# LambdaLabsML/distributed-training-guide

Measured on AMD Instinct MI355X. Metric: tokens/sec/GPU for Llama-style causal LM at 1/2/4/8 MI355X; peak HBM per GPU, higher is better.
Workload: dtype bf16; 1 GPU; model=llama-3-8b, global_batch=24, seq_len=1024, parallelism=single

## Files before the change

### distributed_training_guide_amd/_hip/attention_bwd.hip

```cpp
#include "attention_common.h"
#include "launchers.h"

template <int D>
__global__ void __launch_bounds__(256) attn_delta_kernel(
    const short* __restrict__ dout, const short* __restrict__ o,
    float* __restrict__ delta, int B, int S, int Hq) {
  const int grp = threadIdx.x >> 4;
  const int gl = threadIdx.x & 15;
  int64_t nrows = (int64_t)B * S * Hq;
  for (int64_t row = (int64_t)blockIdx.x * 16 + grp; row < nrows;
       row += (int64_t)gridDim.x * 16) {
    const short* dp = dout + row * D;
    const short* op = o + row * D;
    float s = 0.f;
#pragma unroll
    for (int i = gl * 8; i < D; i += 16 * 8) {
      bf16x8 dv = *reinterpret_cast<const bf16x8*>(dp + i);
      bf16x8 ov = *reinterpret_cast<const bf16x8*>(op + i);
#pragma unroll
      for (int j = 0; j < 8; ++j) s += bf2f(dv[j]) * bf2f(ov[j]);
    }
#pragma unroll
    for (int off = 1; off < 16; off <<= 1) s += __shfl_xor(s, off, WAVE);
    if (gl == 0) {
      int h = (int)(row % Hq);
      int64_t bs = row / Hq;
      int sp = (int)(bs % S);
      int b = (int)(bs / S);
      delta[((int64_t)b * Hq + h) * S + sp] = s;
    }
  }
}

template <int D, bool DOC>
__global__ void __launch_bounds__(256, 2) attn_dkdv_kernel(
    const short* __restrict__ dout, const short* __restrict__ q,
    const short* __restrict__ k, const short* __restrict__ v,
    const float* __restrict__ lse, const float* __restrict__ delta,
    short* __restrict__ dk, short* __restrict__ dv, int B, int S, int Hq,
    int Hkv, float scale, const int* __restrict__ doc_end) {
  static_assert(D == 64 || D == 128, "head dim must be 64 or 128");
  __shared__ short q_lds[2][64 * D];
  __shared__ short do_lds[2][64 * D];
  __shared__ __attribute__((aligned(16))) float lse_lds[2][64];
  __shared__ __attribute__((aligned(16))) float del_lds[2][64];

  const int nkt = (S + 63) / 64;
  const int group = Hq / Hkv;

  const GroupBlock gb = xcd_remap(blockIdx.x, B * Hkv, nkt);
  const int b = gb.gid / Hkv;
  const int hkv = gb.gid % Hkv;
  const int kt = gb.within;

  const int tid = threadIdx.x;
  const int wid = tid >> 6;
  const int lane = tid & (WAVE - 1);
  const int l15 = lane & 15;
  const int lg = lane >> 4;

  const int kv0 = kt * 64 + wid * 16;
  constexpr int nd16 = D >> 4, nkc = D >> 5;
  const float c2 = scale * LOG2E;
  const int64_t strideS_q = (int64_t)Hq * D;
  const int64_t strideS_kv = (int64_t)Hkv * D;
// ... 130 lines not shown
    for (int dt = 0; dt < nd16; ++dt) {
#pragma unroll
      for (int kc = 0; kc < 2; ++kc) {
        bf16x8 dofr = tr16_frag_st(dol, kc * 32 + lg * 8, dt * 16, l15);
        bf16x8 qfr = tr16_frag_st(ql, kc * 32 + lg * 8, dt * 16, l15);
        dvacc[dt] = mfma16(__builtin_bit_cast(bf16x8, pk_p[kc]), dofr,
                           dvacc[dt]);
        dkacc[dt] = mfma16(__builtin_bit_cast(bf16x8, pk_ds[kc]), qfr,
                           dkacc[dt]);
      }
    }
    __builtin_amdgcn_s_setprio(0);
    __syncthreads();
  }

#pragma unroll
  for (int r = 0; r < 4; ++r) {
    int keyw = kv0 + lg * 4 + r;
    if (keyw >= S) continue;
    short* dkp = dk + ((int64_t)b * S * Hkv + (int64_t)keyw * Hkv + hkv) * D;
    short* dvp = dv + ((int64_t)b * S * Hkv + (int64_t)keyw * Hkv + hkv) * D;
#pragma unroll
    for (int dt = 0; dt < nd16; ++dt) {
      dkp[dt * 16 + l15] = f2bf(dkacc[dt][r]);
      dvp[dt * 16 + l15] = f2bf(dvacc[dt][r]);
    }
  }
}

template <int D, bool DOC>
__global__ void __launch_bounds__(256, 2) attn_dq_kernel(
    const short* __restrict__ dout, const short* __restrict__ q,
    const short* __restrict__ k, const short* __restrict__ v,
    const float* __restrict__ lse, const float* __restrict__ delta,
    short* __restrict__ dq, int B, int S, int Hq, int Hkv, float scale,
    const int* __restrict__ doc_start) {
  static_assert(D == 64 || D == 128, "head dim must be 64 or 128");
  __shared__ short k_lds[2][KVBLK * D];
  __shared__ short v_lds[2][KVBLK * D];

  const int ntq = (S + QBLK - 1) / QBLK;
  const int gqa = Hq / Hkv;
  const int bpg = gqa * ntq;

  const GroupBlock gb = xcd_remap(blockIdx.x, B * Hkv, bpg);
  const int b = gb.gid / Hkv;
  const int hkv = gb.gid % Hkv;
  const int h = hkv * gqa + gb.within / ntq;
  const int qtile = gb.within % ntq;

  const int tid = threadIdx.x;
  const int wid = tid >> 6;
  const int lane = tid & (WAVE - 1);
  const int l15 = lane & 15;
  const int lg = lane >> 4;

  const int q0 = qtile * QBLK;
  const int rowb[2] = {qgroup_row(q0, wid, 0), qgroup_row(q0, wid, 1)};
  constexpr int nd16 = D >> 4, nkc = D >> 5;
  const float c2 = scale * LOG2E;
  const int64_t strideS_q = (int64_t)Hq * D;
  const int64_t strideS_kv = (int64_t)Hkv * D;
  const short* qb = q + ((int64_t)b * S * Hq + h) * D;
  const short* dob = dout + ((int64_t)b * S * Hq + h) * D;
  const short* kb = k + ((int64_t)b * S * Hkv + hkv) * D;
  const short* vb = v + ((int64_t)b * S * Hkv + hkv) * D;
  const float* lseb = lse + ((int64_t)b * Hq + h) * S;
  const float* delb = delta + ((int64_t)b * Hq + h) * S;

  bf16x8 qf[2][nkc], dof[2][nkc];
  float lse_r[2], del_r[2];
#pragma unroll
  for (int nq = 0; nq < 2; ++nq) {
    int qrow = rowb[nq] + l15;
    int qrc = qrow < S ? qrow : S - 1;
    const short* qp = qb + (int64_t)qrc * strideS_q + lg * 8;
    const short* dop = dob + (int64_t)qrc * strideS_q + lg * 8;
#pragma unroll
    for (int c = 0; c < nkc; ++c) {
      qf[nq][c] = *reinterpret_cast<const bf16x8*>(qp + c * 32);
      dof[nq][c] = *reinterpret_cast<const bf16x8*>(dop + c * 32);
    }
    lse_r[nq] = lseb[qrc] * LOG2E;
    del_r[nq] = delb[qrc] * scale;
  }

  f32x4 dqacc[nd16][2];
#pragma unroll
  for (int dt = 0; dt < nd16; ++dt)
#pragma unroll
    for (int nq = 0; nq < 2; ++nq) dqacc[dt][nq] = {0.f, 0.f, 0.f, 0.f};

  const int kv_end = min(S, q0 + QBLK);
  const int ntiles = (kv_end + KVBLK - 1) / KVBLK;
  int dstart[2], dsmax[2];
  const int t0 =
      doc_window<DOC>(doc_start, b, S, q0, wid, l15, dstart, dsmax);

  auto stage_kv = [&](int t, int buf) {
    stage_tile_pair<D>(kb, vb, strideS_kv, t * KVBLK, S, k_lds[buf],
                       v_lds[buf], wid, lane);
  };
  stage_kv(t0, 0);
  __syncthreads();

  for (int t = t0; t < ntiles; ++t) {
    const int kv0 = t * KVBLK;
    const int buf = tile_buf(t, t0);
    if (t + 1 < ntiles) stage_kv(t + 1, buf ^ 1);

    {
      const bool smask = (kv_end < kv0 + KVBLK);
      u32x4 pk_ds[2][2];
      const short* kl = k_lds[buf];
      const short* vl = v_lds[buf];
      __builtin_amdgcn_s_setprio(1);
#pragma unroll
// ... 31 lines not shown
              const int keyr = kv0 + koff + r;
              if (keyr > qrow || keyr >= S || qrow >= S ||
                  (DOC && keyr < dstart[nq]))
                e[r] = -INFINITY;
            }
          }
#pragma unroll
          for (int r = 0; r < 4; ++r)
            ds[r] = __builtin_amdgcn_exp2f(e[r]) *
                    __builtin_fmaf(dv[r], scale, -del_r[nq]);
          pk_ds[nq][kc][rp + 0] = cvt_pk_bf16(ds[0], ds[1]);
          pk_ds[nq][kc][rp + 1] = cvt_pk_bf16(ds[2], ds[3]);
        }
      }

#pragma unroll
      for (int dt = 0; dt < nd16; ++dt) {
#pragma unroll
        for (int kc = 0; kc < 2; ++kc) {
          bf16x8 kfr = tr16_frag_st(kl, kc * 32 + lg * 8, dt * 16, l15);
          dqacc[dt][0] = mfma16(__builtin_bit_cast(bf16x8, pk_ds[0][kc]),
                                kfr, dqacc[dt][0]);
          dqacc[dt][1] = mfma16(__builtin_bit_cast(bf16x8, pk_ds[1][kc]),
                                kfr, dqacc[dt][1]);
        }
      }
      __builtin_amdgcn_s_setprio(0);
    }
    __syncthreads();
  }

#pragma unroll
  for (int nq = 0; nq < 2; ++nq) {
#pragma unroll
    for (int r = 0; r < 4; ++r) {
      int qrow = rowb[nq] + lg * 4 + r;
      if (qrow >= S) continue;
      short* dqp = dq + ((int64_t)b * S * Hq + (int64_t)qrow * Hq + h) * D;
#pragma unroll
      for (int dt = 0; dt < nd16; ++dt) {
        dqp[dt * 16 + l15] = f2bf(dqacc[dt][nq][r]);
      }
    }
  }
}

namespace {
template <int D, bool DOC>
void bwd_launch(const short* dout, const short* q, const short* k,
                const short* v, const short* o, const float* lse,
                float* delta, short* dq, short* dk, short* dv,
                const int* doc_start, const int* doc_end, int B, int S,
                int Hq, int Hkv, float scale, hipStream_t stream) {
  int64_t nrows = (int64_t)B * S * Hq;
  int64_t dwant = (nrows + 15) / 16;
  int dgrid = (int)(dwant < 2048 ? (dwant < 1 ? 1 : dwant) : 2048);
  hipLaunchKernelGGL(attn_delta_kernel<D>, dim3(dgrid), dim3(256), 0, stream,
                     dout, o, delta, B, S, Hq);
  int nkt = (S + 63) / 64;
  hipLaunchKernelGGL((attn_dkdv_kernel<D, DOC>),
                     dim3((uint32_t)((int64_t)B * Hkv * nkt)), dim3(256), 0,
                     stream, dout, q, k, v, lse, delta, dk, dv, B, S, Hq, Hkv,
                     scale, doc_end);
  int ntq = (S + QBLK - 1) / QBLK;
  hipLaunchKernelGGL((attn_dq_kernel<D, DOC>),
                     dim3((uint32_t)((int64_t)B * Hq * ntq)), dim3(256), 0,
                     stream, dout, q, k, v, lse, delta, dq, B, S, Hq, Hkv,
                     scale, doc_start);
}
}

extern "C" void attn_bwd_launch(const void* dout, const void* q, const void* k,
                                const void* v, const void* o, const float* lse,
                                float* delta, void* dq, void* dk, void* dv,
                                const int* doc_start, const int* doc_end,
                                int B, int S, int Hq, int Hkv, int D,
                                float scale, hipStream_t stream) {
  const bool doc = doc_start != nullptr;
  auto fn = doc ? (D == 64 ? bwd_launch<64, true> : bwd_launch<128, true>)
                : (D == 64 ? bwd_launch<64, false> : bwd_launch<128, false>);
  fn((const short*)dout, (const short*)q, (const short*)k, (const short*)v,
     (const short*)o, lse, delta, (short*)dq, (short*)dk, (short*)dv,
     doc_start, doc_end, B, S, Hq, Hkv, scale, stream);
}
```

### distributed_training_guide_amd/_hip/bindings.cpp

```cpp
#include <torch/extension.h>
#include <c10/hip/HIPStream.h>
#include <hip/hip_runtime.h>

#include "launchers.h"

namespace {

inline hipStream_t cur_stream() {
  return c10::hip::getCurrentHIPStream().stream();
}

#define CHECK_BF16_CONTIG(t)                                          \
  TORCH_CHECK((t).is_cuda(), #t " must be on the GPU");               \
  TORCH_CHECK((t).dtype() == torch::kBFloat16, #t " must be bf16");   \
  TORCH_CHECK((t).is_contiguous(), #t " must be contiguous")

#define CHECK_ROPE_TABLES(cos, sin, x, D)                                  \
  TORCH_CHECK((D) % 2 == 0, "rope head dim must be even");                 \
  TORCH_CHECK((cos).is_cuda() && (cos).device() == (x).device() &&         \
                  (sin).is_cuda() && (sin).device() == (x).device(),       \
              "rope tables must be on " #x "'s device");                   \
  TORCH_CHECK((cos).dtype() == torch::kFloat &&                            \
                  (sin).dtype() == torch::kFloat,                          \
              "rope tables must be f32");                                  \
// ... 197 lines not shown
  TORCH_CHECK(dy.sizes() == c10::IntArrayRef(sizes),
              "dy must have gu's shape with the last dim halved");
  TORCH_CHECK(dy.device() == gu.device(), "dy must be on gu's device");
  auto dgu = torch::empty_like(gu);
  silu_mul_bwd_launch(dy.data_ptr(), gu.data_ptr(), dgu.data_ptr(),
                      gu.numel() / I2, I, cur_stream());
  return dgu;
}

torch::Tensor embedding_fwd(torch::Tensor table, torch::Tensor ids) {
  CHECK_BF16_CONTIG(table);
  TORCH_CHECK(table.dim() == 2, "table must be [V,H]");
  TORCH_CHECK(ids.is_cuda() && ids.device() == table.device(),
              "ids must be on the table's device");
  TORCH_CHECK(ids.dtype() == torch::kLong && ids.is_contiguous());
  const int64_t V = table.size(0);
  const int H = (int)table.size(1);
  auto sizes = ids.sizes().vec();
  sizes.push_back(H);
  auto out = torch::empty(sizes, table.options());
  embed_fwd_launch(table.data_ptr(), ids.data_ptr<int64_t>(),
                   out.data_ptr(), ids.numel(), H, V, cur_stream());
  return out;
}

torch::Tensor embedding_bwd(torch::Tensor dy, torch::Tensor ids, int64_t V) {
  CHECK_BF16_CONTIG(dy);
  TORCH_CHECK(ids.is_cuda() && ids.device() == dy.device(),
              "ids must be on dy's device");
  TORCH_CHECK(ids.dtype() == torch::kLong && ids.is_contiguous());
  TORCH_CHECK(dy.dim() >= 1 && V > 0, "dy must be [..., H] and V positive");
  const int H = (int)dy.size(-1);
  TORCH_CHECK(dy.numel() == ids.numel() * H, "dy/ids shape mismatch");
  auto acc = torch::empty({V, (int64_t)H},
                          dy.options().dtype(torch::kFloat));
  auto dtable = torch::empty({V, (int64_t)H}, dy.options());
  embed_bwd_launch(dy.data_ptr(), ids.data_ptr<int64_t>(),
                   acc.data_ptr<float>(), dtable.data_ptr(), ids.numel(), H,
                   V, cur_stream());
  return dtable;
}

std::vector<torch::Tensor> layernorm_fwd(torch::Tensor x, torch::Tensor w,
                                         torch::Tensor b, double eps) {
  CHECK_BF16_CONTIG(x);
  CHECK_BF16_CONTIG(w);
  CHECK_BF16_CONTIG(b);
  const int H = (int)x.size(-1);
  const int64_t nrows = x.numel() / H;
  auto y = torch::empty_like(x);
  auto opts = x.options().dtype(torch::kFloat);
  auto mu = torch::empty({nrows}, opts);
  auto rstd = torch::empty({nrows}, opts);
  ln_fwd_launch(x.data_ptr(), w.data_ptr(), b.data_ptr(), y.data_ptr(),
                mu.data_ptr<float>(), rstd.data_ptr<float>(), nrows, H,
                (float)eps, cur_stream());
  return {y, mu, rstd};
}

std::vector<torch::Tensor> layernorm_bwd(torch::Tensor dy, torch::Tensor x,
                                         torch::Tensor w, torch::Tensor mu,
                                         torch::Tensor rstd) {
  CHECK_BF16_CONTIG(dy);
  CHECK_BF16_CONTIG(x);
  const int H = (int)x.size(-1);
  const int64_t nrows = x.numel() / H;
  const int nblocks = (int)std::min<int64_t>(nrows, 2048);
  auto dx = torch::empty_like(x);
  auto dw = torch::empty_like(w);
  auto db = torch::empty_like(w);
  auto dw_partial = alloc_partials(nblocks, H, x);
  auto db_partial = alloc_partials(nblocks, H, x);
// ... 31 lines not shown
  const int B = (int)logits.size(0), S = (int)logits.size(1),
            V = (int)logits.size(2);
  const int64_t nrows = (int64_t)B * S_out;
  auto loss = torch::empty({nrows}, logits.options().dtype(torch::kFloat));
  auto lse = torch::empty({nrows}, logits.options().dtype(torch::kFloat));
  ce_fwd_launch(logits.data_ptr(), labels.data_ptr<int64_t>(),
                loss.data_ptr<float>(), lse.data_ptr<float>(), nrows, S,
                (int)S_out, V, ignore_index, cur_stream());
  return {loss, lse};
}

std::vector<torch::Tensor> ce_fwd_sharded(torch::Tensor logits,
                                          torch::Tensor labels, int64_t S_out,
                                          int64_t vocab_start,
                                          int64_t ignore_index) {
  CHECK_CE_INPUTS(logits, labels, S_out);
  const int B = (int)logits.size(0), S = (int)logits.size(1),
            V = (int)logits.size(2);
  const int64_t nrows = (int64_t)B * S_out;
  auto opts = logits.options().dtype(torch::kFloat);
  auto maxout = torch::empty({nrows}, opts);
  auto sumout = torch::empty({nrows}, opts);
  auto gathered = torch::empty({nrows}, opts);
  ce_fwd_sharded_launch(logits.data_ptr(), labels.data_ptr<int64_t>(),
                        maxout.data_ptr<float>(), sumout.data_ptr<float>(),
                        gathered.data_ptr<float>(), nrows, S, (int)S_out, V,
                        vocab_start, ignore_index, cur_stream());
  return {maxout, sumout, gathered};
}

torch::Tensor ce_bwd(torch::Tensor logits, torch::Tensor labels,
                     torch::Tensor lse, double scale, int64_t S_out,
                     int64_t vocab_start, int64_t ignore_index, bool sharded,
                     c10::optional<torch::Tensor> scale_t = c10::nullopt) {
  CHECK_CE_INPUTS(logits, labels, S_out);
  const int B = (int)logits.size(0), S = (int)logits.size(1),
            V = (int)logits.size(2);
  const int64_t nrows = (int64_t)B * S_out;
  TORCH_CHECK(lse.is_cuda() && lse.device() == logits.device() &&
                  lse.dtype() == torch::kFloat && lse.is_contiguous() &&
                  lse.numel() == nrows,
              "lse must be a contiguous f32 [B*S_out] on the logits' device");
  const float* sp = nullptr;
  if (scale_t.has_value()) {
    TORCH_CHECK(scale_t->dtype() == torch::kFloat && scale_t->is_cuda() &&
                scale_t->numel() == 1, "scale_t must be a cuda f32 scalar");
    sp = scale_t->data_ptr<float>();
  }
  auto dlogits = (S_out == S) ? torch::empty_like(logits)
                              : torch::zeros_like(logits);
  ce_bwd_launch(logits.data_ptr(), labels.data_ptr<int64_t>(),
                lse.data_ptr<float>(), dlogits.data_ptr(), (float)scale, sp,
                nrows, S, (int)S_out, V, vocab_start, ignore_index,
                sharded ? 1 : 0, cur_stream());
  return dlogits;
}

void adamw_step(torch::Tensor descs, int64_t nchunks, double lr, double beta1,
                double beta2, double eps, double wd, int64_t step) {
  TORCH_CHECK(descs.is_cuda() && descs.dtype() == torch::kLong &&
              descs.is_contiguous());
  const float bc1 = 1.0f - std::pow((float)beta1, (float)step);
  const float bc2 = 1.0f - std::pow((float)beta2, (float)step);
  adamw_launch(descs.data_ptr(), (int)nchunks, (float)lr, (float)beta1,
               (float)beta2, (float)eps, (float)wd, 1.0f / bc1, 1.0f / bc2,
               cur_stream());
}

#define CHECK_DESCS(descs, nchunks)                                        \
  TORCH_CHECK((descs).is_cuda() && (descs).dtype() == torch::kLong &&      \
              (descs).is_contiguous());                                    \
  TORCH_CHECK((nchunks) >= 0 && (descs).numel() >= 7 * (nchunks),          \
              "descriptor table shorter than nchunks")

#define CHECK_SQ_TOTAL(t, descs)                                           \
  TORCH_CHECK((t).is_cuda() && (t).dtype() == torch::kFloat &&             \
              (t).numel() == 1 && (t).device() == (descs).device(),        \
              #t " must be a cuda f32 scalar on the descriptors' device")

void adamw_step_clipped(torch::Tensor descs, int64_t nchunks, double lr,
                        double beta1, double beta2, double eps, double wd,
                        int64_t step, torch::Tensor sq_total,
                        double max_norm) {
// ... 138 lines not shown
                       scale);
}
std::vector<torch::Tensor> attn_bwd_doc(torch::Tensor dout, torch::Tensor q,
                                        torch::Tensor k, torch::Tensor v,
                                        torch::Tensor o, torch::Tensor lse,
                                        torch::Tensor doc_start,
                                        torch::Tensor doc_end, double scale) {
  return attn_bwd_impl(dout, q, k, v, o, lse, doc_start, doc_end, scale);
}

}

PYBIND11_MODULE(TORCH_EXTENSION_NAME, m) {
  m.def("rmsnorm_fwd", &rmsnorm_fwd);
  m.def("rmsnorm_bwd", &rmsnorm_bwd);
  m.def("rope", &rope);
  m.def("add_rmsnorm_fwd", &add_rmsnorm_fwd);
  m.def("add_rmsnorm_bwd", &add_rmsnorm_bwd);
  m.def("qkv_rope_fwd", &qkv_rope_fwd);
  m.def("qkv_rope_bwd", &qkv_rope_bwd);
  m.def("silu_mul_fwd", &silu_mul_fwd);
  m.def("silu_mul_bwd", &silu_mul_bwd);
  m.def("embedding_fwd", &embedding_fwd);
  m.def("embedding_bwd", &embedding_bwd);
  m.def("layernorm_fwd", &layernorm_fwd);
  m.def("layernorm_bwd", &layernorm_bwd);
  m.def("gelu_fwd", &gelu_fwd);
  m.def("gelu_bwd", &gelu_bwd);
  m.def("ce_fwd", &ce_fwd);
  m.def("ce_fwd_sharded", &ce_fwd_sharded);
  m.def("ce_bwd", &ce_bwd, py::arg("logits"), py::arg("labels"),
        py::arg("lse"), py::arg("scale"), py::arg("S_out"),
        py::arg("vocab_start"), py::arg("ignore_index"),
        py::arg("sharded"), py::arg("scale_t") = c10::nullopt);
  m.def("adamw_step", &adamw_step);
  m.def("adamw_step_clipped", &adamw_step_clipped);
  m.def("grad_sqsum", &grad_sqsum);
  m.def("grad_scale_", &grad_scale_);
  m.def("attn_fwd", &attn_fwd);
  m.def("attn_bwd", &attn_bwd);
  m.def("attn_fwd_doc", &attn_fwd_doc);
  m.def("attn_bwd_doc", &attn_bwd_doc);
}
```

### distributed_training_guide_amd/_hip/cross_entropy.hip

```cpp
#include "common.h"
#include "launchers.h"

template <bool SHARDED>
__global__ void __launch_bounds__(256) ce_fwd_kernel(
    const short* __restrict__ logits, const int64_t* __restrict__ labels,
    float* __restrict__ loss, float* __restrict__ lse,
    float* __restrict__ maxout,
    float* __restrict__ sumout,
    float* __restrict__ gathered,
    int64_t nrows, int S_logits, int S_out, int V,
    int64_t vocab_start, int64_t ignore_index) {
  __shared__ float scratch[8];
  for (int64_t r = blockIdx.x; r < nrows; r += gridDim.x) {
    int64_t b = r / S_out;
    int64_t s = r % S_out;
    const short* xr = logits + (b * S_logits + s) * V;
    int64_t label = labels[b * S_logits + s + (S_logits - S_out)];
    float m = -INFINITY, sum = 0.0f;
    for (int i = threadIdx.x * 8; i < V; i += blockDim.x * 8) {
      s16x8 v;
      if (i + 8 <= V) v = *reinterpret_cast<const s16x8*>(xr + i);
      else { for (int j = 0; j < 8; ++j) v[j] = (i + j < V) ? xr[i + j] : (short)0xff80;  }
#pragma unroll
      for (int j = 0; j < 8; ++j) {
// ... 3 lines not shown
        sum += __expf(f - m);
      }
    }
    float gm = block_reduce_max(m, scratch);
    sum = (m == -INFINITY) ? 0.0f : sum * __expf(m - gm);
    sum = block_reduce_sum(sum, scratch);
    if (threadIdx.x == 0) {
      if (SHARDED) {
        float g = -INFINITY;
        int64_t local = label - vocab_start;
        if (label != ignore_index && local >= 0 && local < V)
          g = bf2f(xr[local]);
        maxout[r] = gm;
        sumout[r] = sum;
        gathered[r] = g;
      } else {
        if (label == ignore_index) {
          loss[r] = 0.0f;
          lse[r] = -INFINITY;
        } else {
          DTGA_KERNEL_ASSERT(label >= 0 && label < V);
          float l = gm + __logf(sum);
          lse[r] = l;
          loss[r] = l - bf2f(xr[label]);
        }
      }
    }
    __syncthreads();
  }
}

template <bool SHARDED>
__global__ void __launch_bounds__(256) ce_bwd_kernel(
    const short* __restrict__ logits, const int64_t* __restrict__ labels,
    const float* __restrict__ lse, short* __restrict__ dlogits, float scale,
    const float* __restrict__ scale_ptr,
    int64_t nrows, int S_logits, int S_out, int V,
    int64_t vocab_start, int64_t ignore_index) {
  if (scale_ptr != nullptr) scale = scale_ptr[0];
  for (int64_t r = blockIdx.x; r < nrows; r += gridDim.x) {
    int64_t b = r / S_out;
    int64_t s = r % S_out;
    const short* xr = logits + (b * S_logits + s) * V;
    short* dxr = dlogits + (b * S_logits + s) * V;
    int64_t label = labels[b * S_logits + s + (S_logits - S_out)];
    float l = lse[r];
    bool ignored = (label == ignore_index) || (l == -INFINITY);
    if (!SHARDED) DTGA_KERNEL_ASSERT(ignored || (label >= 0 && label < V));
    int64_t local = label - vocab_start;
    for (int i = threadIdx.x * 8; i < V; i += blockDim.x * 8) {
      if (i + 8 <= V) {
        s16x8 v = *reinterpret_cast<const s16x8*>(xr + i);
        s16x8 o;
#pragma unroll
        for (int j = 0; j < 8; ++j) {
          float p = ignored ? 0.0f : __expf(bf2f(v[j]) - l);
          if (!ignored && (int64_t)(i + j) == local) p -= 1.0f;
          o[j] = f2bf(scale * p);
        }
        *reinterpret_cast<s16x8*>(dxr + i) = o;
      } else {
        for (int j = 0; i + j < V; ++j) {
          float p = ignored ? 0.0f : __expf(bf2f(xr[i + j]) - l);
          if (!ignored && (int64_t)(i + j) == local) p -= 1.0f;
          dxr[i + j] = f2bf(scale * p);
        }
      }
    }
// ... 42 lines not shown
```

### distributed_training_guide_amd/_hip/embedding.hip

```cpp
#include "common.h"
#include "launchers.h"

__global__ void __launch_bounds__(256) embed_fwd_kernel(
    const short* __restrict__ table, const int64_t* __restrict__ ids,
    short* __restrict__ out, int64_t nrows, int H, int64_t V) {
  const int wave = threadIdx.x / WAVE;
  const int lane = threadIdx.x % WAVE;
  const int waves = blockDim.x / WAVE;
  for (int64_t r = (int64_t)blockIdx.x * waves + wave; r < nrows;
       r += (int64_t)gridDim.x * waves) {
    int64_t id = ids[r];
    DTGA_KERNEL_ASSERT(id >= 0 && id < V);
    const short* src = table + id * H;
    short* dst = out + r * H;
    if ((H & 7) == 0) {
      for (int i = lane * 8; i < H; i += WAVE * 8)
        *reinterpret_cast<s16x8*>(dst + i) =
            *reinterpret_cast<const s16x8*>(src + i);
    } else {
      for (int i = lane; i < H; i += WAVE) dst[i] = src[i];
    }
  }
}

__global__ void __launch_bounds__(256) embed_bwd_scatter_kernel(
    const short* __restrict__ dy, const int64_t* __restrict__ ids,
    float* __restrict__ acc, int64_t nrows, int H, int64_t V) {
  const int wave = threadIdx.x / WAVE;
  const int lane = threadIdx.x % WAVE;
  const int waves = blockDim.x / WAVE;
  for (int64_t r = (int64_t)blockIdx.x * waves + wave; r < nrows;
       r += (int64_t)gridDim.x * waves) {
    int64_t id = ids[r];
    DTGA_KERNEL_ASSERT(id >= 0 && id < V);
    const short* src = dy + r * H;
    float* dst = acc + id * H;
    if ((H & 3) == 0) {
      for (int i = lane * 4; i < H; i += WAVE * 4) {
        s16x4 v = *reinterpret_cast<const s16x4*>(src + i);
#pragma unroll
        for (int j = 0; j < 4; ++j) atomicAdd(dst + i + j, bf2f(v[j]));
      }
    } else {
      for (int i = lane; i < H; i += WAVE) atomicAdd(dst + i, bf2f(src[i]));
    }
  }
}

__global__ void __launch_bounds__(256) f32_to_bf16_kernel(
    const float* __restrict__ src, short* __restrict__ dst, int64_t n) {
  for (int64_t i = ((int64_t)blockIdx.x * blockDim.x + threadIdx.x) * 4;
       i < n; i += (int64_t)gridDim.x * blockDim.x * 4) {
    if (i + 4 <= n) {
      f32x4 v = *reinterpret_cast<const f32x4*>(src + i);
      s16x4 o;
#pragma unroll
      for (int j = 0; j < 4; ++j) o[j] = f2bf(v[j]);
      *reinterpret_cast<s16x4*>(dst + i) = o;
    } else {
      for (int64_t j = i; j < n; ++j) dst[j] = f2bf(src[j]);
    }
  }
}

extern "C" {
void embed_fwd_launch(const void* table, const int64_t* ids, void* out,
                      int64_t nrows, int H, int64_t V, hipStream_t s) {
  int waves = 4;
  int64_t blocks = (nrows + waves - 1) / waves;
  int grid = (int)(blocks < 8192 ? (blocks < 1 ? 1 : blocks) : 8192);
  hipLaunchKernelGGL(embed_fwd_kernel, dim3(grid), dim3(256), 0, s,
                     (const short*)table, ids, (short*)out, nrows, H, V);
}
void embed_bwd_launch(const void* dy, const int64_t* ids, float* acc,
                      void* dtable, int64_t nrows, int H, int64_t V,
                      hipStream_t s) {
  hipMemsetAsync(acc, 0, (size_t)V * H * sizeof(float), s);
  int waves = 4;
  int64_t blocks = (nrows + waves - 1) / waves;
  int grid = (int)(blocks < 8192 ? (blocks < 1 ? 1 : blocks) : 8192);
  hipLaunchKernelGGL(embed_bwd_scatter_kernel, dim3(grid), dim3(256), 0, s,
                     (const short*)dy, ids, acc, nrows, H, V);
  int64_t n = V * (int64_t)H;
  int64_t cblocks = (n / 4 + 255) / 256;
  int cgrid = (int)(cblocks < 1 ? 1 : cblocks < 8192 ? cblocks : 8192);
  hipLaunchKernelGGL(f32_to_bf16_kernel, dim3(cgrid), dim3(256), 0, s,
                     acc, (short*)dtable, n);
}
}
```

### distributed_training_guide_amd/_hip/launchers.h

```cpp
#pragma once
#include <hip/hip_runtime.h>
#include <stdint.h>

#define COLSUM_RY 16

extern "C" {
void colsum_launch(float* partial, void* out, int nblocks, int H,
                   hipStream_t s);

void rmsnorm_fwd_launch(const void* x, const void* w, void* y, void* rstd,
                        int64_t nrows, int H, float eps, hipStream_t s);
void rmsnorm_bwd_launch(const void* dy, const void* x, const void* w,
                        const void* rstd, void* dx, float* dw_partial,
                        void* dw, int nblocks, int64_t nrows, int H,
                        hipStream_t s);
void add_rmsnorm_fwd_launch(const void* res, const void* delta, const void* w,
                            void* res_out, void* y, void* rstd, int64_t nrows,
                            int H, float eps, hipStream_t s);
void add_rmsnorm_bwd_launch(const void* dy, const void* dres_out,
                            const void* x, const void* w, const void* rstd,
                            void* dx, float* dw_partial, void* dw,
                            int nblocks, int64_t nrows, int H,
                            hipStream_t s);

void ln_fwd_launch(const void* x, const void* w, const void* b, void* y,
                   float* mu, float* rstd, int64_t nrows, int H, float eps,
                   hipStream_t s);
void ln_bwd_launch(const void* dy, const void* x, const void* w,
                   const float* mu, const float* rstd, void* dx,
                   float* dw_partial, float* db_partial, void* dw, void* db,
                   int nblocks, int64_t nrows, int H, hipStream_t s);
void gelu_fwd_launch(const void* x, void* y, int64_t n, hipStream_t s);
void gelu_bwd_launch(const void* dy, const void* x, void* dx, int64_t n,
                     hipStream_t s);

void rope_launch(const void* x, void* y, const float* cs, const float* sn,
                 const int* positions, int64_t total_rows, int S, int H, int D,
                 int backward, hipStream_t stream);
void qkv_rope_fwd_launch(const void* qkv, void* q, void* k, void* v,
                         const float* cs, const float* sn,
                         const int* positions, int64_t BS, int S, int Hq,
                         int Hkv, int D, hipStream_t stream);
void qkv_rope_bwd_launch(const void* dq, const void* dk, const void* dv,
                         void* dqkv, const float* cs, const float* sn,
                         const int* positions, int64_t BS, int S, int Hq,
                         int Hkv, int D, hipStream_t stream);

void silu_mul_fwd_launch(const void* gu, void* y, int64_t nrows, int I,
                         hipStream_t s);
void silu_mul_bwd_launch(const void* dy, const void* gu, void* dgu,
                         int64_t nrows, int I, hipStream_t s);

void embed_fwd_launch(const void* table, const int64_t* ids, void* out,
                      int64_t nrows, int H, int64_t V, hipStream_t s);
void embed_bwd_launch(const void* dy, const int64_t* ids, float* acc,
                      void* dtable, int64_t nrows, int H, int64_t V,
                      hipStream_t s);

void ce_fwd_launch(const void* logits, const int64_t* labels, float* loss,
                   float* lse, int64_t nrows, int S_logits, int S_out, int V,
                   int64_t ignore_index, hipStream_t st);
void ce_fwd_sharded_launch(const void* logits, const int64_t* labels,
                           float* maxout, float* sumout, float* gathered,
                           int64_t nrows, int S_logits, int S_out, int V,
                           int64_t vocab_start, int64_t ignore_index,
                           hipStream_t st);
void ce_bwd_launch(const void* logits, const int64_t* labels, const float* lse,
                   void* dlogits, float scale, const float* scale_ptr,
                   int64_t nrows, int S_logits, int S_out, int V,
                   int64_t vocab_start, int64_t ignore_index, int sharded,
                   hipStream_t st);

void adamw_launch(const void* descs, int nchunks, float lr, float beta1,
                  float beta2, float eps, float wd, float inv_bc1,
                  float inv_bc2, hipStream_t s);
void adamw_launch_clipped(const void* descs, int nchunks, float lr,
                          float beta1, float beta2, float eps, float wd,
                          float inv_bc1, float inv_bc2, const float* sq_total,
                          float max_norm, hipStream_t s);
void grad_sqsum_launch(const void* descs, int nchunks, float* partials,
                       float* out, int slot, hipStream_t s);
void grad_scale_launch(const void* descs, int nchunks, const float* sq_total,
                       float max_norm, hipStream_t s);

void attn_fwd_launch(const void* q, const void* k, const void* v, void* o,
                     float* lse, const int* doc_start, int B, int S, int Hq,
                     int Hkv, int D, float scale, hipStream_t stream);
void attn_bwd_launch(const void* dout, const void* q, const void* k,
                     const void* v, const void* o, const float* lse,
                     float* delta, void* dq, void* dk, void* dv,
// ... 4 lines not shown
```

### distributed_training_guide_amd/_hip/silu_mul.hip

```cpp
#include "common.h"
#include "launchers.h"

__global__ void __launch_bounds__(256) silu_mul_fwd_kernel(
    const short* __restrict__ gu, short* __restrict__ y, int64_t nrows,
    int I) {
  const int gwave = (blockIdx.x * blockDim.x + threadIdx.x) / WAVE;
  const int nwaves = gridDim.x * blockDim.x / WAVE;
  const int lane = threadIdx.x & (WAVE - 1);
  for (int64_t row = gwave; row < nrows; row += nwaves) {
    const short* g = gu + row * (2 * (int64_t)I);
    const short* u = g + I;
    short* yr = y + row * (int64_t)I;
    for (int i = lane * 8; i < I; i += WAVE * 8) {
      s16x8 gv = *reinterpret_cast<const s16x8*>(g + i);
      s16x8 uv = *reinterpret_cast<const s16x8*>(u + i);
      s16x8 o;
#pragma unroll
      for (int j = 0; j < 8; ++j) {
        float x = bf2f(gv[j]);
        float sig = 1.0f / (1.0f + __expf(-x));
        o[j] = f2bf(x * sig * bf2f(uv[j]));
      }
      *reinterpret_cast<s16x8*>(yr + i) = o;
    }
  }
}

__global__ void __launch_bounds__(256) silu_mul_bwd_kernel(
    const short* __restrict__ dy, const short* __restrict__ gu,
    short* __restrict__ dgu, int64_t nrows, int I) {
  const int gwave = (blockIdx.x * blockDim.x + threadIdx.x) / WAVE;
  const int nwaves = gridDim.x * blockDim.x / WAVE;
  const int lane = threadIdx.x & (WAVE - 1);
  for (int64_t row = gwave; row < nrows; row += nwaves) {
    const short* dyr = dy + row * (int64_t)I;
    const short* g = gu + row * (2 * (int64_t)I);
    const short* u = g + I;
    short* dg = dgu + row * (2 * (int64_t)I);
    short* du = dg + I;
    for (int i = lane * 8; i < I; i += WAVE * 8) {
      s16x8 dv = *reinterpret_cast<const s16x8*>(dyr + i);
      s16x8 gv = *reinterpret_cast<const s16x8*>(g + i);
      s16x8 uv = *reinterpret_cast<const s16x8*>(u + i);
      s16x8 og, ou;
#pragma unroll
      for (int j = 0; j < 8; ++j) {
        float x = bf2f(gv[j]);
        float sig = 1.0f / (1.0f + __expf(-x));
        float sx = x * sig;
        float d = bf2f(dv[j]);
        ou[j] = f2bf(d * sx);
        og[j] = f2bf(d * bf2f(uv[j]) * sig * (1.0f + x * (1.0f - sig)));
      }
      *reinterpret_cast<s16x8*>(dg + i) = og;
      *reinterpret_cast<s16x8*>(du + i) = ou;
    }
// ... 21 lines not shown
```

### distributed_training_guide_amd/ops/embedding.py

```python
import torch
import torch.nn as nn
import torch.nn.functional as F

from .._ext import ext, use_hip


class _EmbeddingFn(torch.autograd.Function):
    @staticmethod
    def forward(ctx, ids, weight):
        ctx.save_for_backward(ids)
        ctx.V = weight.shape[0]
        return ext().embedding_fwd(weight, ids)

    @staticmethod
    def backward(ctx, dy):
        (ids,) = ctx.saved_tensors
        dtable = ext().embedding_bwd(dy.contiguous(), ids, ctx.V)
        return None, dtable


class Embedding(nn.Module):

    def __init__(self, num_embeddings: int, embedding_dim: int, device=None,
                 dtype=None):
        super().__init__()
        self.num_embeddings = num_embeddings
        self.embedding_dim = embedding_dim
        self.weight = nn.Parameter(torch.empty(
            num_embeddings, embedding_dim, device=device, dtype=dtype))

    def reset_parameters(self):
        with torch.no_grad():
            if not self.weight.is_meta:
                self.weight.normal_()

    def forward(self, ids):
        import os

        if (use_hip(self.weight)
                and not os.environ.get("DTGA_TORCH_EMBED")
                and not torch.are_deterministic_algorithms_enabled()):
            return _EmbeddingFn.apply(ids.contiguous(), self.weight)
        return F.embedding(ids, self.weight)

    def extra_repr(self):
        return f"{self.num_embeddings}, {self.embedding_dim}"
```

### distributed_training_guide_amd/ops/fused_linear_ce.py

```python
import os

import torch

from .._ext import ext
from .cross_entropy import IGNORE_INDEX
from .reference import cross_entropy_ref


def _shifted_flat_labels(labels: torch.Tensor) -> torch.Tensor:
    B, S = labels.shape
    flat = labels.reshape(-1)
    out = torch.empty_like(flat)
    out[: B * S - 1] = flat[1:]
    out[B * S - 1:].fill_(IGNORE_INDEX)
    out.view(B, S)[:, S - 1].fill_(IGNORE_INDEX)
    return out.contiguous()


class _FusedLinearCEFn(torch.autograd.Function):
    @staticmethod
    def forward(ctx, x, weight, labels, chunk_rows, keep_logits):
        B, S, H = x.shape
        x2 = x.reshape(B * S, H)
        N = B * S
        shifted = _shifted_flat_labels(labels)
        n_valid = (shifted != IGNORE_INDEX).sum().clamp_min(1)
        logits = None
        if keep_logits:
            logits = torch.matmul(x2, weight.t())
            loss_rows, lse = ext().ce_fwd(logits.unsqueeze(0),
                                          shifted.unsqueeze(0), N,
                                          IGNORE_INDEX)
            loss_sum = loss_rows.sum()
        else:
            lse = torch.empty(N, dtype=torch.float32, device=x.device)
            loss_sum = torch.zeros((), dtype=torch.float32, device=x.device)
            wt = weight.t()
            for r0 in range(0, N, chunk_rows):
                r1 = min(r0 + chunk_rows, N)
                logits_c = torch.matmul(x2[r0:r1], wt)
                lc, lse_c = ext().ce_fwd(logits_c.unsqueeze(0),
                                         shifted[r0:r1].unsqueeze(0), r1 - r0,
                                         IGNORE_INDEX)
                loss_sum += lc.sum()
                lse[r0:r1] = lse_c
        if keep_logits:
            ctx.save_for_backward(x2, weight, shifted, lse, n_valid, logits)
        else:
            ctx.save_for_backward(x2, weight, shifted, lse, n_valid)
        ctx.chunk_rows = chunk_rows
        ctx.in_shape = (B, S, H)
        ctx.keep_logits = keep_logits
        return loss_sum / n_valid

    @staticmethod
    def backward(ctx, dloss):
        if ctx.keep_logits:
            x2, weight, shifted, lse, n_valid, logits = ctx.saved_tensors
        else:
            x2, weight, shifted, lse, n_valid = ctx.saved_tensors
            logits = None
        B, S, H = ctx.in_shape
        V = weight.shape[0]
        N = B * S
        scale_t = (dloss.detach() / n_valid).to(torch.float32) \
            .reshape(1).contiguous()
        dx2 = torch.empty_like(x2)
        one_chunk = ctx.chunk_rows >= N
        dw32 = None if one_chunk else torch.zeros(
            V, H, dtype=torch.float32, device=x2.device)
        dw = None
        wt = weight.t()
        for r0 in range(0, N, ctx.chunk_rows):
            r1 = min(r0 + ctx.chunk_rows, N)
            L = r1 - r0
            logits_c = (logits[r0:r1] if logits is not None
                        else torch.matmul(x2[r0:r1], wt))
            dlogits_c = ext().ce_bwd(logits_c.unsqueeze(0),
                                     shifted[r0:r1].unsqueeze(0),
                                     lse[r0:r1], 0.0, L, 0, IGNORE_INDEX,
                                     False, scale_t).squeeze(0)
            del logits_c
            torch.matmul(dlogits_c, weight, out=dx2[r0:r1])
            if one_chunk:
                dw = torch.matmul(dlogits_c.t(), x2[r0:r1])
            else:
                dw32.add_(torch.matmul(dlogits_c.t(), x2[r0:r1]))
        if dw is None:
            dw = dw32.to(weight.dtype)
        return (dx2.view(B, S, H), dw, None, None, None)


def fused_causal_lm_loss(x: torch.Tensor, weight: torch.Tensor,
                         labels: torch.Tensor,
                         chunk_rows: int | None = None) -> torch.Tensor:
    if not x.is_cuda:
        logits = torch.matmul(x, weight.t())
        return cross_entropy_ref(logits, labels, IGNORE_INDEX)
    mode = os.environ.get("DTGA_CE_MODE", "auto")
    if mode == "unfused":
        from .cross_entropy import causal_lm_loss

        return causal_lm_loss(torch.matmul(x, weight.t()), labels)
    if chunk_rows is None:
        chunk_rows = int(os.environ.get("DTGA_CE_CHUNK", "8192"))
    if mode == "semi":
        keep = True
    elif mode == "fused":
        keep = False
    else:
        logits_bytes = x.numel() // x.shape[-1] * weight.shape[0] * 2
        free, _ = torch.cuda.mem_get_info(x.device)
        keep = free > 4 * logits_bytes
    return _FusedLinearCEFn.apply(x.contiguous(), weight,
# ... 2 lines not shown
```

Measured before the change: 24120 tokens/s.

## Fuse attention delta into dq kernel, sort-based embedding backward, in-place CE grads

Several independent changes land together. The attention backward drops the separate delta kernel: the dq kernel now computes rowsum(dO*O) itself and writes delta, and it launches before dkdv. The embedding backward replaces fp32 atomic scatter plus a conversion pass with a sort of the ids and a per-id segmented reduction straight to bf16, and it is now used even when deterministic algorithms are enabled. Cross-entropy backward writes gradients in place into the logits buffer, which saves allocations and memory at the cost of disallowing a second backward in semi mode. The SiLU-mul forward loop is also unrolled by two.

```diff
diff --git a/distributed_training_guide_amd/_hip/attention_bwd.hip b/distributed_training_guide_amd/_hip/attention_bwd.hip
--- a/distributed_training_guide_amd/_hip/attention_bwd.hip
+++ b/distributed_training_guide_amd/_hip/attention_bwd.hip
@@ -1,36 +1,5 @@
 #include "attention_common.h"
 #include "launchers.h"
-
-template <int D>
-__global__ void __launch_bounds__(256) attn_delta_kernel(
-    const short* __restrict__ dout, const short* __restrict__ o,
-    float* __restrict__ delta, int B, int S, int Hq) {
-  const int grp = threadIdx.x >> 4;
-  const int gl = threadIdx.x & 15;
-  int64_t nrows = (int64_t)B * S * Hq;
-  for (int64_t row = (int64_t)blockIdx.x * 16 + grp; row < nrows;
-       row += (int64_t)gridDim.x * 16) {
-    const short* dp = dout + row * D;
-    const short* op = o + row * D;
-    float s = 0.f;
-#pragma unroll
-    for (int i = gl * 8; i < D; i += 16 * 8) {
-      bf16x8 dv = *reinterpret_cast<const bf16x8*>(dp + i);
-      bf16x8 ov = *reinterpret_cast<const bf16x8*>(op + i);
-#pragma unroll
-      for (int j = 0; j < 8; ++j) s += bf2f(dv[j]) * bf2f(ov[j]);
-    }
-#pragma unroll
-    for (int off = 1; off < 16; off <<= 1) s += __shfl_xor(s, off, WAVE);
-    if (gl == 0) {
-      int h = (int)(row % Hq);
-      int64_t bs = row / Hq;
-      int sp = (int)(bs % S);
-      int b = (int)(bs / S);
-      delta[((int64_t)b * Hq + h) * S + sp] = s;
-    }
-  }
-}
 
 template <int D, bool DOC>
 __global__ void __launch_bounds__(256, 2) attn_dkdv_kernel(
@@ -227,9 +196,9 @@
 __global__ void __launch_bounds__(256, 2) attn_dq_kernel(
     const short* __restrict__ dout, const short* __restrict__ q,
     const short* __restrict__ k, const short* __restrict__ v,
-    const float* __restrict__ lse, const float* __restrict__ delta,
-    short* __restrict__ dq, int B, int S, int Hq, int Hkv, float scale,
-    const int* __restrict__ doc_start) {
+    const short* __restrict__ o, const float* __restrict__ lse,
+    float* __restrict__ delta, short* __restrict__ dq, int B, int S, int Hq,
+    int Hkv, float scale, const int* __restrict__ doc_start) {
   static_assert(D == 64 || D == 128, "head dim must be 64 or 128");
   __shared__ short k_lds[2][KVBLK * D];
   __shared__ short v_lds[2][KVBLK * D];
@@ -260,11 +229,12 @@
   const short* dob = dout + ((int64_t)b * S * Hq + h) * D;
   const short* kb = k + ((int64_t)b * S * Hkv + hkv) * D;
   const short* vb = v + ((int64_t)b * S * Hkv + hkv) * D;
+  const short* ob = o + ((int64_t)b * S * Hq + h) * D;
   const float* lseb = lse + ((int64_t)b * Hq + h) * S;
-  const float* delb = delta + ((int64_t)b * Hq + h) * S;
+  float* delb = delta + ((int64_t)b * Hq + h) * S;
 
   bf16x8 qf[2][nkc], dof[2][nkc];
-  float lse_r[2], del_r[2];
+  float lse_r[2], del_r[2], dkeep[2];
 #pragma unroll
   for (int nq = 0; nq < 2; ++nq) {
     int qrow = rowb[nq] + l15;
@@ -277,7 +247,23 @@
       dof[nq][c] = *reinterpret_cast<const bf16x8*>(dop + c * 32);
     }
     lse_r[nq] = lseb[qrc] * LOG2E;
-    del_r[nq] = delb[qrc] * scale;
+  }
+#pragma unroll
+  for (int nq = 0; nq < 2; ++nq) {
+    int qrow = rowb[nq] + l15;
+    int qrc = qrow < S ? qrow : S - 1;
+    const short* op = ob + (int64_t)qrc * strideS_q + lg * 8;
+    float dsum = 0.f;
+#pragma unroll
+    for (int c = 0; c < nkc; ++c) {
+      const bf16x8 of = *reinterpret_cast<const bf16x8*>(op + c * 32);
+#pragma unroll
+      for (int j = 0; j < 8; ++j) dsum += bf2f(dof[nq][c][j]) * bf2f(of[j]);
+    }
+    dsum += __shfl_xor(dsum, 16, WAVE);
+    dsum += __shfl_xor(dsum, 32, WAVE);
+    dkeep[nq] = dsum;
+    del_r[nq] = dsum * scale;
   }
 
   f32x4 dqacc[nd16][2];
@@ -375,6 +361,12 @@
 
 #pragma unroll
   for (int nq = 0; nq < 2; ++nq) {
+    const int qrow = rowb[nq] + l15;
+    if (lg == 0 && qrow < S) delb[qrow] = dkeep[nq];
+  }
+
+#pragma unroll
+  for (int nq = 0; nq < 2; ++nq) {
 #pragma unroll
     for (int r = 0; r < 4; ++r) {
       int qrow = rowb[nq] + lg * 4 + r;
@@ -395,21 +387,16 @@
                 float* delta, short* dq, short* dk, short* dv,
                 const int* doc_start, const int* doc_end, int B, int S,
                 int Hq, int Hkv, float scale, hipStream_t stream) {
-  int64_t nrows = (int64_t)B * S * Hq;
-  int64_t dwant = (nrows + 15) / 16;
-  int dgrid = (int)(dwant < 2048 ? (dwant < 1 ? 1 : dwant) : 2048);
-  hipLaunchKernelGGL(attn_delta_kernel<D>, dim3(dgrid), dim3(256), 0, stream,
-                     dout, o, delta, B, S, Hq);
+  int ntq = (S + QBLK - 1) / QBLK;
+  hipLaunchKernelGGL((attn_dq_kernel<D, DOC>),
+                     dim3((uint32_t)((int64_t)B * Hq * ntq)), dim3(256), 0,
+                     stream, dout, q, k, v, o, lse, delta, dq, B, S, Hq, Hkv,
+                     scale, doc_start);
   int nkt = (S + 63) / 64;
   hipLaunchKernelGGL((attn_dkdv_kernel<D, DOC>),
                      dim3((uint32_t)((int64_t)B * Hkv * nkt)), dim3(256), 0,
                      stream, dout, q, k, v, lse, delta, dk, dv, B, S, Hq, Hkv,
                      scale, doc_end);
-  int ntq = (S + QBLK - 1) / QBLK;
-  hipLaunchKernelGGL((attn_dq_kernel<D, DOC>),
-                     dim3((uint32_t)((int64_t)B * Hq * ntq)), dim3(256), 0,
-                     stream, dout, q, k, v, lse, delta, dq, B, S, Hq, Hkv,
-                     scale, doc_start);
 }
 }
 
diff --git a/distributed_training_guide_amd/_hip/bindings.cpp b/distributed_training_guide_amd/_hip/bindings.cpp
--- a/distributed_training_guide_amd/_hip/bindings.cpp
+++ b/distributed_training_guide_amd/_hip/bindings.cpp
@@ -253,12 +253,14 @@
   TORCH_CHECK(dy.dim() >= 1 && V > 0, "dy must be [..., H] and V positive");
   const int H = (int)dy.size(-1);
   TORCH_CHECK(dy.numel() == ids.numel() * H, "dy/ids shape mismatch");
-  auto acc = torch::empty({V, (int64_t)H},
-                          dy.options().dtype(torch::kFloat));
-  auto dtable = torch::empty({V, (int64_t)H}, dy.options());
-  embed_bwd_launch(dy.data_ptr(), ids.data_ptr<int64_t>(),
-                   acc.data_ptr<float>(), dtable.data_ptr(), ids.numel(), H,
-                   V, cur_stream());
+  auto sorted_perm = torch::sort(ids.reshape({-1}), true,
+                                 0, false);
+  auto sorted = std::get<0>(sorted_perm).contiguous();
+  auto perm = std::get<1>(sorted_perm).contiguous();
+  auto dtable = torch::zeros({V, (int64_t)H}, dy.options());
+  embed_bwd_launch(dy.data_ptr(), sorted.data_ptr<int64_t>(),
+                   perm.data_ptr<int64_t>(), dtable.data_ptr(), ids.numel(),
+                   H, V, cur_stream());
   return dtable;
 }
 
@@ -356,7 +358,8 @@
 torch::Tensor ce_bwd(torch::Tensor logits, torch::Tensor labels,
                      torch::Tensor lse, double scale, int64_t S_out,
                      int64_t vocab_start, int64_t ignore_index, bool sharded,
-                     c10::optional<torch::Tensor> scale_t = c10::nullopt) {
+                     c10::optional<torch::Tensor> scale_t = c10::nullopt,
+                     c10::optional<torch::Tensor> out = c10::nullopt) {
   CHECK_CE_INPUTS(logits, labels, S_out);
   const int B = (int)logits.size(0), S = (int)logits.size(1),
             V = (int)logits.size(2);
@@ -371,8 +374,21 @@
                 scale_t->numel() == 1, "scale_t must be a cuda f32 scalar");
     sp = scale_t->data_ptr<float>();
   }
-  auto dlogits = (S_out == S) ? torch::empty_like(logits)
-                              : torch::zeros_like(logits);
+  torch::Tensor dlogits;
+  if (out.has_value()) {
+    dlogits = *out;
+    CHECK_BF16_CONTIG(dlogits);
+    TORCH_CHECK(dlogits.sizes() == logits.sizes() &&
+                    dlogits.device() == logits.device(),
+                "out must have the shape and device of logits");
+    TORCH_CHECK(!dlogits.is_alias_of(logits) ||
+                    dlogits.data_ptr() == logits.data_ptr(),
+                "out may be logits itself but not a shifted view of it");
+    if (S_out != S) dlogits.narrow(1, S_out, S - S_out).zero_();
+  } else {
+    dlogits = (S_out == S) ? torch::empty_like(logits)
+                           : torch::zeros_like(logits);
+  }
   ce_bwd_launch(logits.data_ptr(), labels.data_ptr<int64_t>(),
                 lse.data_ptr<float>(), dlogits.data_ptr(), (float)scale, sp,
                 nrows, S, (int)S_out, V, vocab_start, ignore_index,
@@ -577,7 +593,8 @@
   m.def("ce_bwd", &ce_bwd, py::arg("logits"), py::arg("labels"),
         py::arg("lse"), py::arg("scale"), py::arg("S_out"),
         py::arg("vocab_start"), py::arg("ignore_index"),
-        py::arg("sharded"), py::arg("scale_t") = c10::nullopt);
+        py::arg("sharded"), py::arg("scale_t") = c10::nullopt,
+        py::arg("out") = c10::nullopt);
   m.def("adamw_step", &adamw_step);
   m.def("adamw_step_clipped", &adamw_step_clipped);
   m.def("grad_sqsum", &grad_sqsum);
diff --git a/distributed_training_guide_amd/_hip/cross_entropy.hip b/distributed_training_guide_amd/_hip/cross_entropy.hip
--- a/distributed_training_guide_amd/_hip/cross_entropy.hip
+++ b/distributed_training_guide_amd/_hip/cross_entropy.hip
@@ -59,8 +59,8 @@
 
 template <bool SHARDED>
 __global__ void __launch_bounds__(256) ce_bwd_kernel(
-    const short* __restrict__ logits, const int64_t* __restrict__ labels,
-    const float* __restrict__ lse, short* __restrict__ dlogits, float scale,
+    const short* logits, const int64_t* __restrict__ labels,
+    const float* __restrict__ lse, short* dlogits, float scale,
     const float* __restrict__ scale_ptr,
     int64_t nrows, int S_logits, int S_out, int V,
     int64_t vocab_start, int64_t ignore_index) {
diff --git a/distributed_training_guide_amd/_hip/embedding.hip b/distributed_training_guide_amd/_hip/embedding.hip
--- a/distributed_training_guide_amd/_hip/embedding.hip
+++ b/distributed_training_guide_amd/_hip/embedding.hip
@@ -23,42 +23,61 @@
   }
 }
 
-__global__ void __launch_bounds__(256) embed_bwd_scatter_kernel(
-    const short* __restrict__ dy, const int64_t* __restrict__ ids,
-    float* __restrict__ acc, int64_t nrows, int H, int64_t V) {
+template <bool VEC>
+__global__ void __launch_bounds__(256) embed_bwd_sorted_kernel(
+    const short* __restrict__ dy, const int64_t* __restrict__ sorted,
+    const int64_t* __restrict__ perm, short* __restrict__ dtable,
+    int64_t nrows, int H, int64_t V) {
   const int wave = threadIdx.x / WAVE;
   const int lane = threadIdx.x % WAVE;
   const int waves = blockDim.x / WAVE;
-  for (int64_t r = (int64_t)blockIdx.x * waves + wave; r < nrows;
-       r += (int64_t)gridDim.x * waves) {
-    int64_t id = ids[r];
+  const int c0 = blockIdx.y * (WAVE * 8) + lane * 8;
+  auto load_row = [&](int64_t r) {
+    s16x8 v;
+    const short* src = dy + r * H + c0;
+    if (VEC) {
+      v = *reinterpret_cast<const s16x8*>(src);
+    } else {
+#pragma unroll
+      for (int e = 0; e < 8; ++e) v[e] = (c0 + e < H) ? src[e] : (short)0;
+    }
+    return v;
+  };
+  for (int64_t i = (int64_t)blockIdx.x * waves + wave; i < nrows;
+       i += (int64_t)gridDim.x * waves) {
+    const int64_t id = sorted[i];
+    if (i > 0 && sorted[i - 1] == id) continue;
     DTGA_KERNEL_ASSERT(id >= 0 && id < V);
-    const short* src = dy + r * H;
-    float* dst = acc + id * H;
-    if ((H & 3) == 0) {
-      for (int i = lane * 4; i < H; i += WAVE * 4) {
-        s16x4 v = *reinterpret_cast<const s16x4*>(src + i);
+    if (id < 0 || id >= V || c0 >= H) continue;
+    float acc[8];
 #pragma unroll
-        for (int j = 0; j < 4; ++j) atomicAdd(dst + i + j, bf2f(v[j]));
-      }
+    for (int e = 0; e < 8; ++e) acc[e] = 0.0f;
+    int64_t j = i;
+    do {
+      int n = 1;
+      while (n < 4 && j + n < nrows && sorted[j + n] == id) ++n;
+      s16x8 v[4];
+#pragma unroll
+      for (int k = 0; k < 4; ++k)
+        if (k < n) v[k] = load_row(perm[j + k]);
+#pragma unroll
+      for (int k = 0; k < 4; ++k)
+        if (k < n) {
+#pragma unroll
+          for (int e = 0; e < 8; ++e) acc[e] += bf2f(v[k][e]);
+        }
+      j += n;
+    } while (j < nrows && sorted[j] == id);
+    short* dst = dtable + id * H + c0;
+    if (VEC) {
+      s16x8 o;
+#pragma unroll
+      for (int e = 0; e < 8; ++e) o[e] = f2bf(acc[e]);
+      *reinterpret_cast<s16x8*>(dst) = o;
     } else {
-      for (int i = lane; i < H; i += WAVE) atomicAdd(dst + i, bf2f(src[i]));
-    }
-  }
-}
-
-__global__ void __launch_bounds__(256) f32_to_bf16_kernel(
-    const float* __restrict__ src, short* __restrict__ dst, int64_t n) {
-  for (int64_t i = ((int64_t)blockIdx.x * blockDim.x + threadIdx.x) * 4;
-       i < n; i += (int64_t)gridDim.x * blockDim.x * 4) {
-    if (i + 4 <= n) {
-      f32x4 v = *reinterpret_cast<const f32x4*>(src + i);
-      s16x4 o;
 #pragma unroll
-      for (int j = 0; j < 4; ++j) o[j] = f2bf(v[j]);
-      *reinterpret_cast<s16x4*>(dst + i) = o;
-    } else {
-      for (int64_t j = i; j < n; ++j) dst[j] = f2bf(src[j]);
+      for (int e = 0; e < 8; ++e)
+        if (c0 + e < H) dst[e] = f2bf(acc[e]);
     }
   }
 }
@@ -72,19 +91,20 @@
   hipLaunchKernelGGL(embed_fwd_kernel, dim3(grid), dim3(256), 0, s,
                      (const short*)table, ids, (short*)out, nrows, H, V);
 }
-void embed_bwd_launch(const void* dy, const int64_t* ids, float* acc,
-                      void* dtable, int64_t nrows, int H, int64_t V,
-                      hipStream_t s) {
-  hipMemsetAsync(acc, 0, (size_t)V * H * sizeof(float), s);
+void embed_bwd_launch(const void* dy, const int64_t* sorted,
+                      const int64_t* perm, void* dtable, int64_t nrows, int H,
+                      int64_t V, hipStream_t s) {
   int waves = 4;
   int64_t blocks = (nrows + waves - 1) / waves;
   int grid = (int)(blocks < 8192 ? (blocks < 1 ? 1 : blocks) : 8192);
-  hipLaunchKernelGGL(embed_bwd_scatter_kernel, dim3(grid), dim3(256), 0, s,
-                     (const short*)dy, ids, acc, nrows, H, V);
-  int64_t n = V * (int64_t)H;
-  int64_t cblocks = (n / 4 + 255) / 256;
-  int cgrid = (int)(cblocks < 1 ? 1 : cblocks < 8192 ? cblocks : 8192);
-  hipLaunchKernelGGL(f32_to_bf16_kernel, dim3(cgrid), dim3(256), 0, s,
-                     acc, (short*)dtable, n);
+  dim3 g(grid, (H + WAVE * 8 - 1) / (WAVE * 8));
+  if ((H & 7) == 0)
+    hipLaunchKernelGGL(embed_bwd_sorted_kernel<true>, g, dim3(256), 0, s,
+                       (const short*)dy, sorted, perm, (short*)dtable, nrows,
+                       H, V);
+  else
+    hipLaunchKernelGGL(embed_bwd_sorted_kernel<false>, g, dim3(256), 0, s,
+                       (const short*)dy, sorted, perm, (short*)dtable, nrows,
+                       H, V);
 }
 }
diff --git a/distributed_training_guide_amd/_hip/launchers.h b/distributed_training_guide_amd/_hip/launchers.h
--- a/distributed_training_guide_amd/_hip/launchers.h
+++ b/distributed_training_guide_amd/_hip/launchers.h
@@ -53,9 +53,9 @@
 
 void embed_fwd_launch(const void* table, const int64_t* ids, void* out,
                       int64_t nrows, int H, int64_t V, hipStream_t s);
-void embed_bwd_launch(const void* dy, const int64_t* ids, float* acc,
-                      void* dtable, int64_t nrows, int H, int64_t V,
-                      hipStream_t s);
+void embed_bwd_launch(const void* dy, const int64_t* sorted,
+                      const int64_t* perm, void* dtable, int64_t nrows, int H,
+                      int64_t V, hipStream_t s);
 
 void ce_fwd_launch(const void* logits, const int64_t* labels, float* loss,
                    float* lse, int64_t nrows, int S_logits, int S_out, int V,
diff --git a/distributed_training_guide_amd/_hip/silu_mul.hip b/distributed_training_guide_amd/_hip/silu_mul.hip
--- a/distributed_training_guide_amd/_hip/silu_mul.hip
+++ b/distributed_training_guide_amd/_hip/silu_mul.hip
@@ -1,5 +1,16 @@
 #include "common.h"
 #include "launchers.h"
+
+__device__ __forceinline__ s16x8 silu_mul_vec(s16x8 gv, s16x8 uv) {
+  s16x8 o;
+#pragma unroll
+  for (int j = 0; j < 8; ++j) {
+    float x = bf2f(gv[j]);
+    float sig = 1.0f / (1.0f + __expf(-x));
+    o[j] = f2bf(x * sig * bf2f(uv[j]));
+  }
+  return o;
+}
 
 __global__ void __launch_bounds__(256) silu_mul_fwd_kernel(
     const short* __restrict__ gu, short* __restrict__ y, int64_t nrows,
@@ -7,21 +18,24 @@
   const int gwave = (blockIdx.x * blockDim.x + threadIdx.x) / WAVE;
   const int nwaves = gridDim.x * blockDim.x / WAVE;
   const int lane = threadIdx.x & (WAVE - 1);
+  constexpr int TRIP = WAVE * 8;
   for (int64_t row = gwave; row < nrows; row += nwaves) {
     const short* g = gu + row * (2 * (int64_t)I);
     const short* u = g + I;
     short* yr = y + row * (int64_t)I;
-    for (int i = lane * 8; i < I; i += WAVE * 8) {
+    int i = lane * 8;
+    for (; i + TRIP < I; i += 2 * TRIP) {
+      s16x8 gv0 = *reinterpret_cast<const s16x8*>(g + i);
+      s16x8 uv0 = *reinterpret_cast<const s16x8*>(u + i);
+      s16x8 gv1 = *reinterpret_cast<const s16x8*>(g + i + TRIP);
+      s16x8 uv1 = *reinterpret_cast<const s16x8*>(u + i + TRIP);
+      *reinterpret_cast<s16x8*>(yr + i) = silu_mul_vec(gv0, uv0);
+      *reinterpret_cast<s16x8*>(yr + i + TRIP) = silu_mul_vec(gv1, uv1);
+    }
+    if (i < I) {
       s16x8 gv = *reinterpret_cast<const s16x8*>(g + i);
       s16x8 uv = *reinterpret_cast<const s16x8*>(u + i);
-      s16x8 o;
-#pragma unroll
-      for (int j = 0; j < 8; ++j) {
-        float x = bf2f(gv[j]);
-        float sig = 1.0f / (1.0f + __expf(-x));
-        o[j] = f2bf(x * sig * bf2f(uv[j]));
-      }
-      *reinterpret_cast<s16x8*>(yr + i) = o;
+      *reinterpret_cast<s16x8*>(yr + i) = silu_mul_vec(gv, uv);
     }
   }
 }
diff --git a/distributed_training_guide_amd/ops/embedding.py b/distributed_training_guide_amd/ops/embedding.py
--- a/distributed_training_guide_amd/ops/embedding.py
+++ b/distributed_training_guide_amd/ops/embedding.py
@@ -38,8 +38,7 @@
         import os
 
         if (use_hip(self.weight)
-                and not os.environ.get("DTGA_TORCH_EMBED")
-                and not torch.are_deterministic_algorithms_enabled()):
+                and not os.environ.get("DTGA_TORCH_EMBED")):
             return _EmbeddingFn.apply(ids.contiguous(), self.weight)
         return F.embedding(ids, self.weight)
 
diff --git a/distributed_training_guide_amd/ops/fused_linear_ce.py b/distributed_training_guide_amd/ops/fused_linear_ce.py
--- a/distributed_training_guide_amd/ops/fused_linear_ce.py
+++ b/distributed_training_guide_amd/ops/fused_linear_ce.py
@@ -51,6 +51,7 @@
         ctx.chunk_rows = chunk_rows
         ctx.in_shape = (B, S, H)
         ctx.keep_logits = keep_logits
+        ctx.logits_consumed = False
         return loss_sum / n_valid
 
     @staticmethod
@@ -65,6 +66,21 @@
         N = B * S
         scale_t = (dloss.detach() / n_valid).to(torch.float32) \
             .reshape(1).contiguous()
+        if logits is not None:
+            if ctx.logits_consumed:
+                raise RuntimeError(
+                    "fused_causal_lm_loss: the saved logits were overwritten "
+                    "with their gradient by the first backward; a second "
+                    "backward through the same graph (retain_graph=True) "
+                    "is not supported in DTGA_CE_MODE=semi")
+            ctx.logits_consumed = True
+            l3 = logits.unsqueeze(0)
+            dlogits = ext().ce_bwd(l3, shifted.unsqueeze(0), lse, 0.0, N, 0,
+                                   IGNORE_INDEX, False, scale_t,
+                                   out=l3).squeeze(0)
+            dx2 = torch.matmul(dlogits, weight)
+            dw = torch.matmul(dlogits.t(), x2)
+            return (dx2.view(B, S, H), dw, None, None, None)
         dx2 = torch.empty_like(x2)
         one_chunk = ctx.chunk_rows >= N
         dw32 = None if one_chunk else torch.zeros(
@@ -74,12 +90,11 @@
         for r0 in range(0, N, ctx.chunk_rows):
             r1 = min(r0 + ctx.chunk_rows, N)
             L = r1 - r0
-            logits_c = (logits[r0:r1] if logits is not None
-                        else torch.matmul(x2[r0:r1], wt))
-            dlogits_c = ext().ce_bwd(logits_c.unsqueeze(0),
-                                     shifted[r0:r1].unsqueeze(0),
+            logits_c = torch.matmul(x2[r0:r1], wt).unsqueeze(0)
+            dlogits_c = ext().ce_bwd(logits_c, shifted[r0:r1].unsqueeze(0),
                                      lse[r0:r1], 0.0, L, 0, IGNORE_INDEX,
-                                     False, scale_t).squeeze(0)
+                                     False, scale_t,
+                                     out=logits_c).squeeze(0)
             del logits_c
             torch.matmul(dlogits_c, weight, out=dx2[r0:r1])
             if one_chunk:
```

Result: no change. 24330 tokens/s (median of 6 runs) (+0.9%).
